# sovrasov/3d-object-detection.pytorch

Hardware: AMD Instinct MI355X
Metric: regression train crops/sec @224^2 bs256 MobileNetV2 (higher is better)
Workload: dtype bf16; 1 GPU; mobilenetv2 9-class Objectron keypoint regression, train step (fwd + l1/add/CE losses + bwd + AdamW), 224x224 crops, per-GPU batch 256; global_batch=256, parallelism=dp1, roofline_sampled_steps=0, rccl_ranks=0

## Files before the change

3d-object-detection.pytorch_amd/csrc/pwconv_wgrad_tr.hip:

```cpp
#include <cstdlib>
#include "pwconv_route.h"

namespace {

__device__ __forceinline__ f32x2 pk_fma_clamp01(f32x2 a, f32x2 b, f32x2 c) {
  f32x2 d;
  asm("v_pk_fma_f32 %0, %1, %2, %3 clamp" : "=v"(d) : "v"(a), "v"(b), "v"(c));
  return d;
}

typedef __attribute__((ext_vector_type(4))) short s16x4;

__device__ __forceinline__ void act_vec8(float* v, int act) {
  switch (act) {
    case T3D_ACT_RELU:
#pragma unroll
      for (int j = 0; j < 8; ++j) v[j] = fmaxf(v[j], 0.f);
      break;
    case T3D_ACT_RELU6:
#pragma unroll
      for (int j = 0; j < 8; ++j) v[j] = __builtin_amdgcn_fmed3f(v[j], 0.f, 6.f);
      break;
    case T3D_ACT_HSWISH:
#pragma unroll
// ... 9 lines not shown
  int per_sample;
  const float *scale, *shift, *se;
  int act, se_after;
  float* dw;
  int M, HW, K, N;
  int yfree, Nz;
  int swap;
  int ptiles, qtiles, rows_per_split, nsplit;
  float* ws;
  const T3dFold* fold;
  const bf16_t* wd;
  const bf16_t* wtr;
  const void *e_res, *e_y;
  void* dx;
  double* stats;
  int nrep;
  long long rstride;
  int unused_[10];
  int assign;
  int gs_ns;
  unsigned mulHW;
};

__device__ __forceinline__ bf16x8 tr_frag(const bf16_t* tile, int rs, int ch0, int lane) {
  const int g = lane >> 4, q = (lane & 15) >> 2, p = lane & 3;
  const bf16_t* a0 = tile + (8 * g + q) * rs + ch0 + 4 * p;
  const s16x4 lo = __builtin_amdgcn_ds_read_tr16_b64_v4i16((s16x4 __attribute__((address_space(3)))*)(a0));
  const s16x4 hi = __builtin_amdgcn_ds_read_tr16_b64_v4i16((s16x4 __attribute__((address_space(3)))*)(a0 + 4 * rs));
  typedef __attribute__((ext_vector_type(8))) short s16x8;
  const s16x8 v = {lo[0], lo[1], lo[2], lo[3], hi[0], hi[1], hi[2], hi[3]};
  return __builtin_bit_cast(bf16x8, v);
}

template <int NTPW, int NTQ, bool SWAP, int G, int D, int GEN, bool YF, int SK = 1, bool DGF = false>
__global__ __launch_bounds__(256 * G) void pw_wgrad_tr_kernel(const WgtArgs a) {
  static_assert(!DGF || (YF && !SWAP), "the fused data gradient exists for the y-free layout only");
  constexpr int PB = 64 * NTPW, QB = 16 * NTQ;
  constexpr int RSP = PB + 8, RSQ = QB + 8;
  constexpr int STEP = 32 * SK;
  extern __shared__ __attribute__((aligned(16))) unsigned char smem[];
  constexpr int BUFE = STEP * (RSP + RSQ);
  const int grp = threadIdx.x >> 8;
  bf16_t* const tiles = reinterpret_cast<bf16_t*>(smem) + grp * 2 * BUFE;
  float* coef = reinterpret_cast<float*>(reinterpret_cast<bf16_t*>(smem) + G * 2 * BUFE);
  constexpr int RSW = PB + 8;
  constexpr int NCOEF = 3 * (SWAP ? QB : PB) + 2 * (SWAP ? PB : QB);
  bf16_t* const wdl = reinterpret_cast<bf16_t*>(coef + ((NCOEF + 3) & ~3));
  double* const dstat = reinterpret_cast<double*>(wdl + (DGF ? QB * RSW : 0));

  const int tid = threadIdx.x & 255, lane = tid & 63, wave = tid >> 6;
  const int P = SWAP ? a.K : a.N, Q = SWAP ? a.N : a.K;
  const int ntiles = a.ptiles * a.qtiles, s8 = a.nsplit & ~7;
  int tile, split;
  {
    const int L = blockIdx.x;
    if (ntiles > 1 && L < ntiles * s8) {
      const int j = L >> 3;
      tile = j % ntiles;
      split = (j / ntiles) * 8 + (L & 7);
    } else {
      const int Lr = ntiles > 1 ? L - ntiles * s8 : L;
      tile = Lr % ntiles;
      split = (ntiles > 1 ? s8 : 0) + Lr / ntiles;
    }
  }
  const int pt = tile / a.qtiles, qt = tile % a.qtiles;
  const int p0 = pt * PB, q0 = qt * QB;
  const int mbeg = split * a.rows_per_split, mend = min(a.M, mbeg + a.rows_per_split);
  constexpr int dyB = SWAP ? QB : PB, aB = SWAP ? PB : QB;
// ... 94 lines not shown
#pragma unroll
            for (int r = 0; r < 4; ++r) {
              const int k = kt * 16 + 4 * lgq_ + r, k2 = qt2 * 16 + lcq_;
              if (k < K && k2 < K) wdl[k * RSW + Nz + k2] = (bf16_t)qa[r];
            }
          }
          __syncthreads();
        }
      if (grp == 0) {
        for (int kb = 0; kb < QB; kb += 16) {
          const int row = tid >> 4, sub = tid & 15, k = kb + row;
          float s2 = 0.f;
          if (k < K)
            for (int n = sub * 8; n < Nz; n += 128) {
              const bf16x8 v = *reinterpret_cast<const bf16x8*>(wtr + (size_t)k * Nz + n);
#pragma unroll
              for (int j = 0; j < 8; ++j) s2 = fmaf(gamma[n + j], (float)v[j], s2);
            }
          s2 = row16_sum(s2);
          if (sub == 0 && k < K) wdl[k * RSW + Nz + K] = (bf16_t)s2;
        }
      }
    }
    for (int i = threadIdx.x; i < 2 * QB; i += 256 * G) dstat[i] = 0.0;
  }
  const bf16_t* __restrict__ dz = reinterpret_cast<const bf16_t*>(a.dz);
  const bf16_t* __restrict__ yy = reinterpret_cast<const bf16_t*>(a.y);
  const bf16_t* __restrict__ xx = reinterpret_cast<const bf16_t*>(a.x);
  const bool plain_a = !a.scale && !a.se && a.act == T3D_ACT_NONE;

  constexpr int dyV = dyB / 8, aV = aB / 8;
  constexpr int ndv = STEP * dyV, nav = STEP * aV;
  constexpr int VDY = (ndv + 255) / 256, VA = (nav + 255) / 256;
  constexpr int NU = DGF ? (STEP / 16) * NTQ : 1, UPW = (NU + 3) / 4;
  struct Epi { bf16x4 res[UPW], xr[UPW]; };
  struct NoMask {};
  struct Regs { bf16x8 rz[VDY], ry[VDY], rx[VA]; Epi e; NoMask okm; };
  Regs rr[D];
  Epi ecur;
  const int lgq = lane >> 4, lcq = lane & 15;
  const bf16_t* __restrict__ eres = reinterpret_cast<const bf16_t*>(a.e_res);
  const bf16_t* __restrict__ eyr = reinterpret_cast<const bf16_t*>(a.e_y);

  auto gload = [&](Regs& R, int m0) {
#pragma unroll
    for (int i = 0; i < VDY; ++i) {
      const int v = min(tid + 256 * i, ndv - 1);
      const int row = v / dyV, m = min(m0 + row, a.M - 1);
      if constexpr (YF) {
        const int n = dy0 + (v % dyV) * 8;
        const bool fromz = n < a.Nz;
        const bf16_t* src = fromz ? dz + (size_t)m * a.Nz + n : xx + (size_t)m * a.K + min(max(n - a.Nz, 0), a.K - 8);
        R.rz[i] = *reinterpret_cast<const bf16x8*>(src);
      } else {
        const int n = min(dy0 + (v % dyV) * 8, a.N - 8);
        R.rz[i] = *reinterpret_cast<const bf16x8*>(dz + (size_t)m * a.N + n);
        R.ry[i] = *reinterpret_cast<const bf16x8*>(yy + (size_t)m * a.N + n);
      }
    }
#pragma unroll
    for (int i = 0; i < VA; ++i) {
      const int v = min(tid + 256 * i, nav - 1);
      const int row = v / aV, k = min(a0c + (v % aV) * 8, a.K - 8), m = min(m0 + row, a.M - 1);
      R.rx[i] = *reinterpret_cast<const bf16x8*>(xx + (size_t)m * a.K + k);
    }
    if constexpr (DGF) {
#pragma unroll
      for (int i = 0; i < UPW; ++i) {
        const int un = min(wave + 4 * i, NU - 1), pt = un / NTQ, kt = un % NTQ;
        const size_t o = (size_t)min(m0 + pt * 16 + lcq, a.M - 1) * a.K + min(kt * 16 + 4 * lgq, a.K - 4);
        if (eres) R.e.res[i] = *reinterpret_cast<const bf16x4*>(eres + o);
        if (eyr) R.e.xr[i] = *reinterpret_cast<const bf16x4*>(eyr + o);
      }
    }
  };
  auto ld8 = [](const float* p, float* o) {
    const float4 q0 = *reinterpret_cast<const float4*>(p), q1 = *reinterpret_cast<const float4*>(p + 4);
    o[0] = q0.x; o[1] = q0.y; o[2] = q0.z; o[3] = q0.w; o[4] = q1.x; o[5] = q1.y; o[6] = q1.z; o[7] = q1.w;
  };
  bf16x8 zero8;
#pragma unroll
  for (int j = 0; j < 8; ++j) zero8[j] = (bf16_t)0.f;
  auto lstore = [&](const Regs& R, int m0, int buf) {
    const auto& rz = R.rz; const auto& ry = R.ry; const auto& rx = R.rx;
    bf16_t* const pb_ = tiles + buf * BUFE;
    bf16_t* const qb_ = pb_ + STEP * RSP;
    bf16_t* dyt = SWAP ? qb_ : pb_;
    bf16_t* at = SWAP ? pb_ : qb_;
    constexpr int rsd = SWAP ? RSQ : RSP, rsa = SWAP ? RSP : RSQ;
#pragma unroll
    for (int i = 0; i < VDY; ++i) {
      const int v = tid + 256 * i;
      if (v < ndv) {
        const int row = v / dyV, cl = (v % dyV) * 8, m = m0 + row;
        const bool ok = m < mend && dy0 + cl < a.N;
        bf16x8 o;
        if constexpr (YF) {
          const int n = dy0 + cl;
          o = rz[i];
          if (n >= a.Nz + a.K) {
            o = zero8;
            if (n == a.Nz + a.K) o[0] = (bf16_t)1.f;
          }
          *reinterpret_cast<bf16x8*>(dyt + row * rsd + cl) = ok ? o : zero8;
          continue;
        }
        float al[8], be[8], ga[8];
        ld8(cdy + dyB + cl, be);
        if constexpr (GEN == 1) {
          if (a.per_sample) {
            const size_t pb = (size_t)(min(m, a.M - 1) / a.HW) * a.N + min(dy0 + cl, a.N - 8);
#pragma unroll
            for (int j = 0; j < 8; ++j) { al[j] = a.alpha[pb + j]; ga[j] = a.gamma[pb + j]; }
          } else {
            ld8(cdy + cl, al);
            ld8(cdy + 2 * dyB + cl, ga);
          }
        } else {
          ld8(cdy + cl, al);
          ld8(cdy + 2 * dyB + cl, ga);
        }
#pragma unroll
        for (int j = 0; j < 8; ++j) o[j] = (bf16_t)fmaf(al[j], (float)rz[i][j], fmaf(be[j], (float)ry[i][j], ga[j]));
        *reinterpret_cast<bf16x8*>(dyt + row * rsd + cl) = ok ? o : zero8;
// ... 30 lines not shown
          }
          if constexpr (GEN == 1) {
            if (a.se) {
              float svv[8];
              {
                const float* se = a.se + (size_t)(min(m, a.M - 1) / a.HW) * a.K + min(a0c + cl, a.K - 8);
#pragma unroll
                for (int j = 0; j < 8; ++j) svv[j] = se[j];
              }
#pragma unroll
              for (int j = 0; j < 8; ++j) {
                float t = fmaf(u[j], sc[j], sh[j]);
                const float sv = svv[j];
                if (!a.se_after) t *= sv;
                t = act_apply(t, a.act);
                if (a.se_after) t *= sv;
                u[j] = t;
              }
              done = true;
            }
          }
          if (c6) {
#pragma unroll
            for (int j = 0; j < 8; j += 2) {
              const f32x2 t = pk_fma_clamp01(f32x2{u[j], u[j + 1]}, f32x2{sc[j], sc[j + 1]}, f32x2{sh[j], sh[j + 1]});
              u[j] = t[0];
              u[j + 1] = t[1];
            }
          } else if (!done) act_affine_vec<8>(u, sc, sh, a.act);
#pragma unroll
          for (int j = 0; j < 8; ++j) o[j] = (bf16_t)u[j];
        }
        *reinterpret_cast<bf16x8*>(at + row * rsa + cl) = ok ? o : zero8;
      }
    }
  };

  f32x4 acc[NTPW][NTQ];
#pragma unroll
  for (int i = 0; i < NTPW; ++i)
#pragma unroll
    for (int j = 0; j < NTQ; ++j) acc[i][j] = f32x4{0.f, 0.f, 0.f, 0.f};
  float st1[UPW][4], st2[UPW][4];
#pragma unroll
  for (int i = 0; i < UPW; ++i)
#pragma unroll
    for (int r = 0; r < 4; ++r) st1[i][r] = st2[i][r] = 0.f;
  auto dgrad_step = [&](const bf16_t* pcur, int m0) {
    bf16_t* __restrict__ dxo = reinterpret_cast<bf16_t*>(a.dx);
#pragma unroll
    for (int i = 0; i < UPW; ++i) {
      const int un = wave + 4 * i;
      if (un < NU) {
        const int pt = un / NTQ, kt = un % NTQ;
        f32x4 d = {0.f, 0.f, 0.f, 0.f};
#pragma unroll
        for (int js = 0; js < PB / 32; ++js) {
          const bf16x8 af = *reinterpret_cast<const bf16x8*>(wdl + (kt * 16 + lcq) * RSW + js * 32 + 8 * lgq);
          const bf16x8 bfr = *reinterpret_cast<const bf16x8*>(pcur + (pt * 16 + lcq) * RSP + js * 32 + 8 * lgq);
          d = __builtin_amdgcn_mfma_f32_16x16x32_bf16(af, bfr, d, 0, 0, 0);
        }
        const int m = m0 + pt * 16 + lcq, k = kt * 16 + 4 * lgq;
        const bool ok = m < mend && k < a.K;
        float v[4] = {d[0], d[1], d[2], d[3]}, yv[4] = {0.f, 0.f, 0.f, 0.f};
        if (eres) {
#pragma unroll
          for (int r = 0; r < 4; ++r) v[r] += (float)ecur.res[i][r];
        }
        bf16x4 o;
#pragma unroll
        for (int r = 0; r < 4; ++r) {
          o[r] = (bf16_t)v[r];
          v[r] = ok ? (float)o[r] : 0.f;
        }
        if (ok) *reinterpret_cast<bf16x4*>(dxo + (size_t)m * a.K + k) = o;
        if (a.stats) {
#pragma unroll
          for (int r = 0; r < 4; ++r) {
            if (eyr) yv[r] = (float)ecur.xr[i][r];
            st1[i][r] += v[r];
            st2[i][r] = fmaf(v[r], eyr ? yv[r] : v[r], st2[i][r]);
          }
        }
      }
    }
  };

  __syncthreads();
  const int nsteps = (mend - mbeg + STEP - 1) / STEP;
  const int niter = (nsteps + G - 1) / G;
  auto step_m = [&](int it) { return mbeg + (it * G + grp) * STEP; };
#pragma unroll
  for (int u = 0; u < D; ++u) gload(rr[u], step_m(u));
  lstore(rr[0], step_m(0), 0);
  if constexpr (DGF) ecur = rr[0].e;
  __syncthreads();
  int buf = 0;
  for (int it0 = 0; it0 < niter; it0 += D) {
#pragma unroll
    for (int u = 0; u < D; ++u) {
      const int it = it0 + u;
      if (it < niter) {
        gload(rr[u], step_m(it + D));
        const bf16_t* pcur = tiles + buf * BUFE;
        const bf16_t* qcur = pcur + STEP * RSP;
#pragma unroll
        for (int kk = 0; kk < SK; ++kk) {
          bf16x8 qf[NTQ];
#pragma unroll
          for (int j = 0; j < NTQ; ++j) qf[j] = tr_frag(qcur + kk * 32 * RSQ, RSQ, j * 16, lane);
#pragma unroll
          for (int i = 0; i < NTPW; ++i) {
            const bf16x8 pf = tr_frag(pcur + kk * 32 * RSP, RSP, (wave + 4 * i) * 16, lane);
#pragma unroll
            for (int j = 0; j < NTQ; ++j) acc[i][j] = __builtin_amdgcn_mfma_f32_16x16x32_bf16(pf, qf[j], acc[i][j], 0, 0, 0);
          }
        }
        if constexpr (DGF) {
          dgrad_step(pcur, step_m(it));
          ecur = rr[(u + 1) % D].e;
// ... 104 lines not shown
  if (sp == 0 && live) dw[(size_t)p * K + q] = assign ? s : dw[(size_t)p * K + q] + s;
}

template <int SG>
__global__ __launch_bounds__(256) void wgrad_reduce_tr_kernel(const float* __restrict__ ws, float* __restrict__ dw, int N, int K,
                                                               int PB, int QB, int qtiles, int tiles, int S, int assign) {
  constexpr int PT = 8 / SG;
  __shared__ float part[8][33];
  const int Qpad = qtiles * QB, nq = (Qpad + 31) / 32;
  const int p0 = (blockIdx.x / nq) * PT, q0 = (blockIdx.x % nq) * 32;
  const int tx = threadIdx.x & 31, rest = threadIdx.x >> 5, sg = rest / PT, pl = rest % PT;
  const size_t stride = (size_t)tiles * PB * QB;
  const int q = q0 + tx, p = p0 + pl;
  float s = 0.f;
  if (p < K && q < N) {
    const float* src = ws + (size_t)((p / PB) * qtiles + q / QB) * (PB * QB) + (size_t)(p % PB) * QB + q % QB;
#pragma unroll 8
    for (int i = sg; i < S; i += SG) s += src[(size_t)i * stride];
  }
  part[rest][tx] = s;
  __syncthreads();
  if (threadIdx.x < 32 * PT) {
    const int pl2 = threadIdx.x % PT, ql = threadIdx.x / PT;
    const int k = p0 + pl2, n = q0 + ql;
    if (k < K && n < N) {
      float t = part[pl2][ql];
#pragma unroll
      for (int g = 1; g < SG; ++g) t += part[g * PT + pl2][ql];
      dw[(size_t)n * K + k] = assign ? t : dw[(size_t)n * K + k] + t;
    }
  }
}

template <int NTPW, int NTQ, bool SWAP, int D, int GEN, bool YF = false, int SK = 1>
int launch_d(WgtArgs& a, hipStream_t st) {
  constexpr int G = 2;
  constexpr int STEP = 32 * SK;
  constexpr int PB = 64 * NTPW, QB = 16 * NTQ;
  const int P = a.swap ? a.K : a.N, Q = a.swap ? a.N : a.K;
  a.ptiles = cdiv(P, PB);
  a.qtiles = cdiv(Q, QB);
  const int tiles = a.ptiles * a.qtiles;
  const int dyB = a.swap ? QB : PB, aB = a.swap ? PB : QB;
  size_t lds = (size_t)G * 2 * STEP * ((PB + 8) + (QB + 8)) * 2 + (size_t)(3 * dyB + 2 * aB) * 4;
  const int tgt_blocks = 256;
  const long long cap_mb = 8;
  int S = (tgt_blocks + tiles - 1) / tiles;
  const long long tile_bytes = (long long)tiles * PB * QB * 4;
  const bool use_ws = g_t3d_ws.ptr && g_t3d_ws.bytes >= tile_bytes;
  if (use_ws) {
    const long long fit = g_t3d_ws.bytes / tile_bytes;
    if (S > fit) S = (int)fit;
  } else {
    const long long flush_cap = (cap_mb << 20) / ((long long)a.N * a.K * 4 + 1);
    if (S > flush_cap) S = (int)(flush_cap < 1 ? 1 : flush_cap);
  }
  const int maxs = cdiv(a.M, STEP * 4 * G);
  if (S > maxs) S = maxs;
  if (S < 1) S = 1;
  a.rows_per_split = cdiv(cdiv(a.M, S), STEP) * STEP;
  S = cdiv(a.M, a.rows_per_split);
  a.gs_ns = 0;
  if constexpr (GEN == 2) {
    const long long ns = a.rows_per_split / a.HW + 2, span = (long long)a.rows_per_split + a.HW;
    if (!a.se || a.per_sample || a.HW < 2 || ns * aB * 4 > 32 * 1024 || span * a.HW >= (1ll << 32)) return launch_d<NTPW, NTQ, SWAP, 1, 1>(a, st);
    a.gs_ns = (int)ns;
    a.mulHW = (unsigned)(((1ull << 32) + a.HW - 1) / a.HW);
    lds = ((lds + 15) & ~(size_t)15) + (size_t)ns * aB * 4;
  }
  a.ws = use_ws ? reinterpret_cast<float*>(g_t3d_ws.ptr) : nullptr;
  if (a.assign && !use_ws && hipMemsetAsync(a.dw, 0, (size_t)a.N * a.K * sizeof(float), st) != hipSuccess) return T3D_ERR_LAUNCH;
  if (lds > 64 * 1024)
    (void)t3d_max_lds((const void*)pw_wgrad_tr_kernel<NTPW, NTQ, SWAP, G, D, GEN, YF, SK, false>, (int)lds);
  a.nsplit = S;
  T3D_LAUNCH_TIMED((pw_wgrad_tr_kernel<NTPW, NTQ, SWAP, G, D, GEN, YF, SK, false>), dim3(tiles * S), dim3(256 * G), lds, st, a);
  if (use_ws) {
#define T3D_WGR(SPV)                                                                                                              \
  do {                                                                                                                            \
    if (SWAP)                                                                                                                     \
      T3D_LAUNCH(wgrad_reduce_tr_kernel<(SPV == 16 ? 8 : SPV)>, dim3(cdiv(a.K, 8 / (SPV == 16 ? 8 : SPV)) * cdiv(a.qtiles * QB, 32)), dim3(256), 0, st, \
                         a.ws, a.dw, a.N, a.K, PB, QB, a.qtiles, tiles, S, a.assign);                                             \
    else                                                                                                                          \
      T3D_LAUNCH(wgrad_reduce_kernel<SPV>, dim3(cdiv(a.N * a.qtiles * QB, 256 / SPV)), dim3(256), 0, st, a.ws, a.dw, a.N, \
                         a.K, PB, QB, a.qtiles, tiles, S, a.assign);                                                              \
  } while (0)
    if (S >= 64) T3D_WGR(16);
    else if (S >= 8) T3D_WGR(4);
    else T3D_WGR(1);
#undef T3D_WGR
  }
  T3D_CHECK_LAUNCH();
  return T3D_OK;
}

template <int NTPW, int NTQ, bool SWAP>
int launch_sw(WgtArgs& a, hipStream_t st) {
  constexpr bool narrow = 64 * NTPW + 16 * NTQ <= 288;
  const bool sk2 = narrow && a.M >= (1 << 20);
  if (a.yfree) {
    if constexpr (SWAP) return T3D_ERR_ARG;
    else {
      if constexpr (narrow)
        if (sk2) return launch_d<NTPW, NTQ, false, 2, false, true, 2>(a, st);
      return launch_d<NTPW, NTQ, false, 2, false, true>(a, st);
    }
  }
  if (a.per_sample) return launch_d<NTPW, NTQ, SWAP, 1, 1>(a, st);
  if (a.se) return launch_d<NTPW, NTQ, SWAP, 2, 2>(a, st);
  if constexpr (narrow)
    if (sk2) return launch_d<NTPW, NTQ, SWAP, 2, false, false, 2>(a, st);
  return launch_d<NTPW, NTQ, SWAP, 2, false>(a, st);
}

template <int NTPW, int NTQ>
int launch_cfg(WgtArgs& a, hipStream_t st) {
  return a.swap ? launch_sw<NTPW, NTQ, true>(a, st) : launch_sw<NTPW, NTQ, false>(a, st);
}

static int choose_and_launch(WgtArgs& a, hipStream_t st) {
  const int M = a.M, K = a.K, N = a.N;
  a.swap = K > N;
  const int P = a.swap ? K : N, Q = a.swap ? N : K;
  const int min_steps = 12;
  auto steps_with = [&](int ntpw, int qb) {
    const int tiles = cdiv(P, 64 * ntpw) * cdiv(Q, qb);
    int S = cdiv(256, tiles);
    if (S < 1) S = 1;
    return M / (S * 2 * 32);
  };
  if (Q <= 16) return (P <= 64 || steps_with(2, 16) < min_steps) ? launch_cfg<1, 1>(a, st) : launch_cfg<2, 1>(a, st);
  if (Q <= 32) {
    if (P <= 64 || steps_with(3, 32) < min_steps) return launch_cfg<1, 2>(a, st);
    return P <= 128 ? launch_cfg<2, 2>(a, st) : launch_cfg<3, 2>(a, st);
  }
// ... 130 lines not shown
```

3d-object-detection.pytorch_amd/torchdet3d/models/engine.py:

```python
import contextlib
import math
import os

import torch

from .. import _native as N
from .arch import Arch

BN_EPS, BN_MOM = 1e-5, 0.1
NREP = 16
FUSED_EVAL_MIN_B = int(os.environ.get('T3D_FUSED_EVAL_MIN_B', '96'))
DW_SLOTS = 512
WORKSPACE_BYTES = 64 << 20
MAIN_WORKSPACE_BYTES = 16 << 20
YFREE_MIN_ELEMS = int(os.environ.get('T3D_YFREE_MIN', 8 << 20))
YFREE_MAX_K = 112
HOOK_MIN = 1 << 20
SE_AFTER_FUSED = None


def _se_after_fused_by_shape(dt, B, HW, C, R):
    if B < 8:
        return False
    if C * R <= 4096:
        return True
    return B >= 16 and B * HW >= 1024


class _BN:
    __slots__ = ('name', 'C', 'gamma', 'beta', 'dgamma', 'dbeta', 'rm', 'rv', 'nbt', 'stats', 'bstats', 'scale',
                 'shift', 'mean', 'invstd', 'alpha', 'bbeta', 'gammac', 'count', 'pro_cache', 'pend', 'desc', 'nrep')


def _nrep_for(C):
    return 16 if C <= 160 else (8 if C <= 640 else 4)


def _concurrent_stream(device, tries=8):
    main = torch.cuda.current_stream(device)
    cands = []
    with torch.cuda.device(device):
        probe = torch.zeros(1, device=device)
        for _ in range(tries):
            st = torch.cuda.Stream(device=device, priority=0)
            cands.append(st)
            e0, e_side, e_main = (torch.cuda.Event(enable_timing=True) for _ in range(3))
            torch.cuda.synchronize(device)
            e0.record(main)
            torch.cuda._sleep(4_000_000)
# ... 32 lines not shown
        self.feat_gain = 1.0
        if self.arch.head == 'conv_bias':
            self.pool = N.POOL['avg']
            self.feat_gain = 2.0 if pooling_mode == 'avg+max' else 1.0
        self.device = torch.device(device)
        assert dtype in (torch.float32, torch.bfloat16, torch.float16)
        self.dtype = dtype
        self.dt = {torch.float32: N.F32, torch.bfloat16: N.BF16, torch.float16: N.F16}[dtype]
        self.esz = 4 if dtype == torch.float32 else 2
        self._share = share
        self._layout()
        self._bufs = {}
        self._packed_dirty = True
        self._packed_version = -1
        self._pack_desc = self._se_pack_desc = None
        self._evdesc = None
        self._dwarena = self._zero_rows = None
        self._zgroups = {'fwd': {}, 'bwd': {}}
        self._zcovered = {'fwd': frozenset(), 'bwd': frozenset()}
        self._zgdesc, self._zdescs = {}, {}
        self._want_taps = None
        self._stop_after = None
        self._tap_res = {}
        self._dropout_calls = 0
        self.seed_rank = 0
        self.saved = None
        self.generation = 0
        self.grad_hook = None
        self._cur_pool_exact = False
        self._side = None
        if self.device.type == 'cuda' and not os.environ.get('T3D_NO_SIDE_STREAM'):
            self._side = _concurrent_stream(self.device)
        self._side_busy = False
        self.persistent_outputs = False
        self.set_input_normalization([0.5931, 0.4690, 0.4229], [0.2471, 0.2214, 0.2157])
        self._fused_eval = True

    def set_input_normalization(self, mean, std):
        self.in_mean = torch.tensor(mean, dtype=torch.float32, device=self.device)
        self.in_istd = 1.0 / torch.tensor(std, dtype=torch.float32, device=self.device)

    def _layout(self):
        a = self.arch
        shapes = a.param_shapes(self.num_classes)
        self.shapes = shapes
        order = [k for k, (s, kind) in shapes.items() if kind == 'param' and not k.startswith('regressors.')]
        off, self.offsets = 0, {}
        for k in order:
            n = int(math.prod(shapes[k][0]))
            self.offsets[k] = (off, n)
            off += (n + 3) // 4 * 4
        F = a.feat_c
        self.offsets['__wreg'] = (off, 9 * 18 * F)
        off += 9 * 18 * F
        self.offsets['__breg'] = (off, 9 * 18 + 2)
        off += 164
        for k in range(9):
            self.offsets[f'regressors.{k}.0.weight'] = (self.offsets['__wreg'][0] + k * 18 * F, 18 * F)
            self.offsets[f'regressors.{k}.0.bias'] = (self.offsets['__breg'][0] + k * 18, 18)
        self.nparams = off
        dev = self.device
        sh = self._share
        assert sh is None or (sh.nparams == off and sh.name == self.name and sh.device == dev)
        self.flat = sh.flat if sh is not None else torch.zeros(off, device=dev)
        self.gflat = sh.gflat if sh is not None else torch.zeros(off, device=dev)
        self.p, self.g = {}, {}
# ... 331 lines not shown
            N.call('t3d_set_main_workspace', N.ptr(ws), MAIN_WORKSPACE_BYTES)
        else:
            N.call('t3d_set_main_workspace', None, 0)

    @contextlib.contextmanager
    def _pass(self, main_scratch=False, workspace=False):
        self._cur_nrep = None
        self._replicas(NREP)
        if workspace:
            N.call('t3d_set_workspace', N.ptr(self._buf('workspace', (WORKSPACE_BYTES,), torch.uint8)), WORKSPACE_BYTES)
        if main_scratch:
            self._main_scratch(True)
        try:
            yield
        finally:
            N.call('t3d_set_reduction_replicas', 1, 0)
            if workspace:
                N.call('t3d_set_dw_slots', 0, None)
            self._pool_exact(False)
            self._cur_nrep = None
            if workspace:
                N.call('t3d_set_workspace', None, 0)
            if main_scratch:
                self._main_scratch(False)

    def forward(self, imgs, cats, train=False, dropout_mask=None, all_heads=False):
        with self._pass(main_scratch=True):
            return self._forward(imgs, cats, train, dropout_mask, all_heads)

    def _forward(self, imgs, cats, train=False, dropout_mask=None, all_heads=False):
        a, st = self.arch, N.stream()
        if train and self.dt == N.F16:
            raise RuntimeError('fp16 storage is an inference-only mode (build the model with storage_dtype bf16 or f32 to train)')
        sv = self._features(imgs, train)
        B = sv['B']
        pooled, cur, yl, prol = sv['pooled'], sv['last_in'], sv['yl'], sv['prol']
        if not all_heads:
            cats = cats.to(self.device, torch.int64).contiguous()
        sv['cats'] = cats
        amax = None
        if self.pool != N.POOL['avg']:
            amax = self._buf('pool_argmax', (B, a.last_c), torch.int32)
        self._c('t3d_pool_fwd', self.dt, N.ptr(yl), prol, self.pool, N.ptr(pooled), N.ptr(amax), B, cur.H * cur.W,
                a.last_c, st, fwd=sv['bnl'])
        sv['pool_argmax'] = amax

        f, fpro = pooled, None
        if a.head == 'linear_bn':
            bnc = self.bns[a.keys.head_bn]
            yc = self._buf('y:cls', (B, a.classifier), torch.float32)
            N.call('t3d_pwconv_fwd', N.F32, N.ptr(pooled), None, N.ptr(self.p[a.keys.head_w]),
                   N.ptr(self.p[a.keys.head_b]), N.ptr(yc), self._st(bnc), B, 1, a.last_c, a.classifier, st)
            fpro = self._bn_fwd(bnc, B, 'hswish')
            self._settle_f(bnc)
            f = yc
        elif a.head == 'conv_bias':
            Fc = a.classifier
            yc = self._buf('y:cls', (B, Fc), torch.float32)
            N.call('t3d_pwconv_fwd', N.F32, N.ptr(pooled), None, N.ptr(self.p[a.keys.head_w]),
                   N.ptr(self.p[a.keys.head_b]), N.ptr(yc), None, B, 1, a.last_c, Fc, st)
            f, fpro = yc, N.prologue(self._const(Fc, 1.0), self._const(Fc, 0.0), None, 'hswish', False)
            sv['head_u'], sv['head_pro'] = yc, fpro
            if self.feat_gain != 1.0:
                f = self._buf('f:gain', (B, Fc), torch.float32)
                N.call('t3d_bn_apply', N.F32, N.ptr(yc), fpro, None, N.ptr(f), B, Fc, st)
                N.call('t3d_bn_apply', N.F32, N.ptr(f), None, N.ptr(f), N.ptr(f), B, Fc, st)
                fpro = None
        ncls = self.num_classes
        keep = self.persistent_outputs
        logits = (self._buf('out:logits', (B, ncls), torch.float32) if keep else torch.empty(B, ncls, device=self.device)) if ncls > 1 else None
        if all_heads:
            kp = self._buf('out:kp_all', (9, B, 18), torch.float32) if keep else torch.empty(9, B, 18, device=self.device)
            N.call('t3d_head_fwd_all', N.ptr(f), fpro, N.ptr(self.wreg), N.ptr(self.breg),
                   N.ptr(self.p['cls_fc.1.weight']) if ncls > 1 else None,
                   N.ptr(self.p['cls_fc.1.bias']) if ncls > 1 else None, N.ptr(kp), N.ptr(logits), B, a.feat_c, ncls, st)
            self.saved = None
            return kp.view(9, B, 9, 2), logits
        mask = None
        if train and ncls > 1:
            mask = dropout_mask
            if mask is None:
                mask = self._buf('dropout', (B, a.feat_c), torch.float32)
                self._dropout_calls += 1
                seed = (torch.initial_seed() + 0x9E3779B97F4A7C15 * self.seed_rank) & ((1 << 64) - 1)
                N.call('t3d_dropout_mask', N.ptr(mask), B * a.feat_c, seed, self._dropout_calls, 0.5, st, slots={3: N.SLOT_DROPOUT})
            else:
                mask = mask.to(self.device, torch.float32).contiguous()
        kp = self._buf('out:kp', (B, 18), torch.float32) if keep else torch.empty(B, 18, device=self.device)
        N.call('t3d_head_fwd', N.ptr(f), fpro, N.ptr(cats), N.ptr(self.wreg), N.ptr(self.breg),
               N.ptr(self.p['cls_fc.1.weight']), N.ptr(self.p['cls_fc.1.bias']), N.ptr(mask), N.ptr(kp),
               N.ptr(logits), B, a.feat_c, ncls, st)
        sv.update(f=f, fpro=fpro, mask=mask, kp=kp)
        assert not any(b.pend[0] for b in self.bns.values()), 'a BatchNorm finalize was never run'
        if train:
            self.generation += 1
            sv['generation'] = self.generation
        self.saved = sv if train else None
        return kp.view(B, 9, 2), logits

    def forward_taps(self, imgs, tap_blocks):
        self._want_taps = set(tap_blocks)
        try:
            with self._pass():
                sv = self._features(imgs, False)
        finally:
            self._want_taps = None
        return {k: (s.t, s.B, s.H, s.W, s.C) for k, s in sv['taps'].items()}

    def _check_train_taps(self, taps):
        a = self.arch
        if a.kind != 'mobilenet' or not taps or min(taps) < 1 or max(taps) > len(a.blocks):
            raise NotImplementedError(f'tapped training pass: taps {sorted(taps)} of {self.name}')
        for k in sorted(taps)[:-1]:
            blk = a.blocks[k]
            if blk.res or not blk.expand:
                why = 'has a skip connection' if blk.res else 'has no expansion'
                raise NotImplementedError(f'tapped training pass: the tap at features.{k} feeds features.{k + 1}, which {why}')

    def forward_taps_train(self, imgs, tap_blocks):
        taps = set(int(k) for k in tap_blocks)
        self._check_train_taps(taps)
# ... 34 lines not shown
        s = sv['taps'][deep]
        M = s.B * s.H * s.W
        dz = self._buf('dz:tap', (M, s.C))
        N.call('t3d_bn_act_bwd', self.dt, N.ptr(dtaps[deep]), N.ptr(s.raw), None, N.ptr(dz), self._bst(s.bn), M, s.C, st)
        self._tap_res = {k: dtaps[k] for k in order[:-1]}
        try:
            for rec in reversed(sv['blocks']):
                dz = self._block_bwd(rec, dz)
                self._maybe_hook(self.offsets[a.keys.blocks[rec['idx']].first][0])
        finally:
            self._tap_res = {}
        self._stem_wgrad(sv, dz, dw32)
        self._flush_dw()
        self._join_side()
        self._maybe_hook(0, force=True)
        assert not any(b.pend[1] for b in self.bns.values()), 'a BatchNorm backward finalize was never run'
        self.saved = None

    def extract_features(self, imgs):
        with self._pass():
            sv = self._features(imgs, False)
        cur, a = sv['last_in'], self.arch
        M = sv['B'] * cur.H * cur.W
        z = torch.empty(M, a.last_c, device=self.device, dtype=self.dtype)
        N.call('t3d_bn_apply', self.dt, N.ptr(sv['yl']), sv['prol'], None, N.ptr(z), M, a.last_c, N.stream())
        return z.float().view(sv['B'], cur.H, cur.W, a.last_c).permute(0, 3, 1, 2).contiguous()

    def _features(self, imgs, train):
        a, st, dt = self.arch, N.stream(), self.dt
        u8 = imgs.dtype == torch.uint8
        assert imgs.is_cuda and imgs.dim() == 4 and ((u8 and imgs.shape[3] == 3) or (imgs.dtype == torch.float32 and imgs.shape[1] == 3))
        imgs = imgs.contiguous()
        self.training = bool(train)
        self._pack()
        if u8:
            B, H, W, _ = imgs.shape
        else:
            B, _, H, W = imgs.shape
        if train:
            self._zero_group('fwd', [[self._statbuf.data_ptr(), self._statbuf.numel() * self._statbuf.element_size()]])
        else:
            self._zero_group('fwd')
            self._eval_affines()
        sv = dict(B=B, imgs=imgs, blocks=[])
        self.saved_blocks = sv['blocks']

        Ho, Wo = (H + 2 - 3) // 2 + 1, (W + 2 - 3) // 2 + 1
        M = B * Ho * Wo
        bn0 = self.bns[a.keys.stem_bn]
        y0 = self._buf('y:stem', (M, a.stem_c))
        col = self._buf('col', (M, 32))
        if u8:
            N.call('t3d_stem_im2col_u8', dt, N.ptr(imgs), N.ptr(self.in_mean), N.ptr(self.in_istd), N.ptr(col), B, H, W, st)
        else:
            N.call('t3d_stem_im2col', dt, N.ptr(imgs), N.ptr(col), B, H, W, st)
        N.call('t3d_pwconv_fwd', dt, N.ptr(col), None, N.ptr(self.w['stem']), None, N.ptr(y0), self._st(bn0),
               M, Ho * Wo, 32, a.stem_c, st, nbytes=M * (32 + a.stem_c) * self.esz)
        pro0 = self._bn_fwd(bn0, M, a.stem_act)
        cur = _Src(y0, pro0, B, Ho, Wo, a.stem_c, raw=y0, bn=bn0, gpro=pro0)
        sv['col'], sv['stem'] = col, cur

        taps = self._want_taps
        for i, blk in enumerate(a.blocks):
            cur = self._block_fwd(i, blk, cur, sv)
            if taps and (i + 1) in taps:
                sv.setdefault('taps', {})[i + 1] = self._resolve(cur)
            if self._stop_after == i + 1:
                return sv

        bnl = self.bns[a.keys.last_bn]
        M = cur.B * cur.H * cur.W
        yl = self._buf('y:last', (M, a.last_c))
        self._pw_from(cur, self.w[a.keys.last_w], yl, bnl, M, cur.H * cur.W, cur.C, a.last_c)
        prol = self._bn_fwd(bnl, M, a.last_act)
        pooled = self._buf('pooled', (B, a.last_c), torch.float32)
        sv.update(last_in=cur, yl=yl, prol=prol, pooled=pooled, HWl=cur.H * cur.W, bnl=bnl)
        return sv

    def _wsel(self, w, plain=True):
        f = self._frag.get(w.data_ptr()) if (plain and self.dt in (N.BF16, N.F16)) else None
        return (self.dt | N.W_FRAG, N.ptr(f)) if f is not None else (self.dt, N.ptr(w))

    def _resolve(self, src):
        if src.zbuf is not None:
            M = src.B * src.H * src.W
            self._c('t3d_bn_apply', self.dt, N.ptr(src.t), src.pro, N.ptr(src.zres), N.ptr(src.zbuf), M, src.C, N.stream(),
                    fwd=src.bn)
            src.t, src.pro, src.zres, src.zbuf = src.zbuf, None, None, None
# ... 147 lines not shown
        if ro is not None and ro.pend[1] and not req:
            self._settle_b(ro)
        if req:
            N.call('t3d_fold_request', N.ptr(self._fold_desc(ro, 1, ro.count)), N.ptr(ro.alpha))
        try:
            self._wgrad_issue(entry, args, kw)
        finally:
            if req and N.lib().t3d_fold_pending():
                raise RuntimeError(f'{entry} left a BatchNorm finalize request unserved (engine / library mismatch)')

    def _wgrad_issue(self, entry, args, kw):
        if self._side is None:
            N.call(entry, *args, N.stream(), **kw)
            return
        self._fork_side()
        if N.timer is None:
            N.call(entry, *args, self._side.cuda_stream, **kw)
        else:
            with torch.cuda.stream(self._side):
                N.call(entry, *args, N.stream(), **kw)
        self._side_busy = True

    def _se_wgrad(self, se, sen, dq, dp, B, C, R):
        self._wgrad(N.ptr(se['m']), N.ptr(se['h']), N.ptr(dq), N.ptr(dp), N.ptr(self.g[sen.se_w1]),
                    N.ptr(self.g[sen.se_b1]), N.ptr(self.g[sen.se_w2]), N.ptr(self.g[sen.se_b2]),
                    B, C, R, entry='t3d_se_bwd_weights')

    def _fork_side(self):
        main = torch.cuda.current_stream()
        self._side.wait_stream(main)
        if N.recorder is not None:
            N.recorder.add_fork(main.cuda_stream, self._side.cuda_stream)

    def _join_side(self):
        if self._side is not None and self._side_busy:
            main = torch.cuda.current_stream()
            main.wait_stream(self._side)
            if N.recorder is not None:
                N.recorder.add_fork(self._side.cuda_stream, main.cuda_stream)
            self._side_busy = False

    def backward(self, dkp, dlogits=None):
        with self._pass(main_scratch=True, workspace=True):
            return self._backward(dkp, dlogits)

    def _clear_backward(self):
        if self._dwarena is None:
            self._dw_arena_init()
        dw32 = self._buf('dstem32', (self.arch.stem_c, 32), torch.float32)
        if self._zero_rows is None:
            rows = [[t.data_ptr(), t.numel() * t.element_size()] for t in (self.gflat, dw32) if t.numel()]
            rows += [[v.data_ptr(), NREP * self.p[k].numel() * 4] for k, v in self._dwviews.items()]
            assert all(r[1] % 16 == 0 for r in rows)
            self._zero_rows = rows
        self._zero_group('bwd', self._zero_rows)
        return dw32

    def _backward(self, dkp, dlogits=None):
        sv = self.saved
        assert sv is not None and 'tap_order' not in sv, 'backward() needs a preceding forward(train=True)'
        a, st, dt, B = self.arch, N.stream(), self.dt, sv['B']
        dw32 = self._clear_backward()
        self._dwpending, self._dwflushed, self._hook_hi = 0, 0, self.gflat.numel()
        dkp = dkp.reshape(B, 18).to(torch.float32).contiguous()
        ncls = self.num_classes
        if ncls > 1:
            assert dlogits is not None
            dlogits = dlogits.to(torch.float32).contiguous()
        else:
            dlogits = None
        F = a.feat_c
        dpre = self._buf('dpre', (B, 18), torch.float32)
        df = self._buf('df', (B, F), torch.float32)
        bnc = self.bns[a.keys.head_bn] if a.head == 'linear_bn' else None
        hstat = None
        if a.head == 'conv_bias':
            hstat = self._buf('head_stats', (2 * F,), torch.float64, zgroup='bwd')
            self._replicas(1)
        N.call('t3d_head_bwd', N.ptr(sv['f']), sv['fpro'], N.ptr(sv['cats']), N.ptr(self.wreg),
               N.ptr(self.p['cls_fc.1.weight']), N.ptr(sv['mask']), N.ptr(sv['kp']), N.ptr(dkp), N.ptr(dlogits),
               N.ptr(dpre), N.ptr(df), self._bst(bnc) if bnc else (N.ptr(hstat) if sv['fpro'] is not None else None),
               None, None, None, None, B, F, ncls, st)
        self._wgrad(N.ptr(sv['f']), sv['fpro'], N.ptr(sv['cats']), N.ptr(sv['mask']), N.ptr(dpre), N.ptr(dlogits),
                    N.ptr(self.dwreg), N.ptr(self.dbreg), N.ptr(self.g['cls_fc.1.weight']), N.ptr(self.g['cls_fc.1.bias']),
                    B, F, ncls, entry='t3d_head_bwd_weights')
        dpooled = df
        if a.head == 'conv_bias':
            yc, pooled, Fc = sv['head_u'], sv['pooled'], a.classifier
            if sv['fpro'] is None:
                du = self._buf('dhead_u', (B, Fc), torch.float32)
                N.call('t3d_bn_act_bwd', N.F32, N.ptr(df), N.ptr(yc), sv['head_pro'], N.ptr(du), N.ptr(hstat), B, Fc, st)
                df = du
            gain, zeros = self._const(Fc, self.feat_gain), self._const(Fc, 0.0)
            bb = N.bnbwd(gain, zeros, zeros, False)
            self._wgrad(N.F32, N.ptr(df), N.ptr(yc), bb, N.ptr(pooled), None, N.ptr(self.g[a.keys.head_w]), B, 1, a.last_c, Fc)
# ... 21 lines not shown
        self.saved = None

    def _backward_backbone(self, sv, dpooled, dw32):
        a, st, dt, B = self.arch, N.stream(), self.dt, sv['B']
        lw = a.keys.last_w
        bnl = self.bns[a.keys.last_bn]
        x = sv['last_in']
        M, HW = B * sv['HWl'], sv['HWl']
        dzl = self._buf('dz:last', (M, a.last_c))
        N.call('t3d_pool_bwd', dt, N.ptr(dpooled), N.ptr(sv['yl']), sv['prol'], self.pool, N.ptr(sv['pool_argmax']),
               N.ptr(dzl), self._bst(bnl), B, HW, a.last_c, st)
        bb = self._bn_bwd(bnl)
        def last_wgrad():
            self._wgrad(dt, N.ptr(dzl), N.ptr(sv['yl']), bb, N.ptr(x.t), x.pro,
                        N.ptr(self.g[lw]), M, HW, x.C, a.last_c, nbytes=M * (x.C + a.last_c) * self.esz,
                        ro=bnl)
        last_wgrad()
        dz = self._pw_dgrad(dzl, sv['yl'], bb, self.wt[lw], x, None, M, HW, x.C, a.last_c, 'dz:lastin', bnl)

        self._maybe_hook(self.offsets[lw][0])
        for rec in reversed(sv['blocks']):
            dz = self._block_bwd(rec, dz)
            self._maybe_hook(self.offsets[a.keys.blocks[rec['idx']].first][0])

        self._stem_wgrad(sv, dz, dw32)

    def _stem_wgrad(self, sv, dz, dw32):
        a, st, dt = self.arch, N.stream(), self.dt
        s0 = sv['stem']
        bn0 = s0.bn
        bb = self._bn_bwd(bn0)
        self._settle_b(bn0)
        M = s0.B * s0.H * s0.W
        self._wgrad(dt, N.ptr(dz), N.ptr(s0.raw), bb, N.ptr(sv['col']), None, N.ptr(dw32),
                    M, s0.H * s0.W, 32, a.stem_c, nbytes=M * (32 + a.stem_c) * self.esz)
        self._flush_dw()
        self._join_side()
        N.call('t3d_copy_cols', N.ptr(dw32), N.ptr(self.g[a.keys.stem_w]), a.stem_c, 32, 27, st)

    def _pw_dgrad(self, dz, y, bb, wt, x, residual, M, HW, K, Nn, tag, bn=None):
        dx = self._buf(tag, (M, K))
        with_stats = x.bn is not None and not x.finished_act
        wd, wp = self._wsel(wt, not bb.per_sample and not (with_stats and x.gpro is not None and x.gpro.se))
        self._c('t3d_pwconv_dgrad', wd, N.ptr(dz), N.ptr(y), bb, wp,
                N.ptr(x.raw) if with_stats else None, x.gpro if with_stats else None,
                N.ptr(residual) if residual is not None else None, N.ptr(dx),
                self._bst(x.bn) if with_stats else None, None, M, HW, K, Nn, N.stream(),
                nbytes=M * (K + Nn) * self.esz, bwd=bn)
        if x.finished_act:
            dx = self._act_bwd(dx, x, tag + ':a')
        return dx

    def _dw_arena_init(self):
        names = [k for k, (sh, kind) in self.shapes.items() if kind == 'param' and len(sh) == 4 and sh[1] == 1 and sh[2] > 1]
        tot = sum(DW_SLOTS * self.p[k].numel() for k in names)
        self._dwarena = torch.zeros(tot, device=self.device, dtype=torch.float32)
        self._dwused = torch.zeros(max(len(names), 1), device=self.device, dtype=torch.int32)
        self._dwviews, self._dwidx, off = {}, {}, 0
        for k in names:
            n = self.p[k].numel()
            self._dwviews[k] = self._dwarena[off:off + DW_SLOTS * n]
            off += DW_SLOTS * n
        self._dworder = list(reversed(names))
        rows = []
        for i, k in enumerate(self._dworder):
            self._dwidx[k] = i
            rows.append([self._dwviews[k].data_ptr(), self.g[k].data_ptr(), self.p[k].numel(), self._dwused[i:i + 1].data_ptr()])
        self._dwdesc = torch.tensor(rows, dtype=torch.int64, device=self.device) if rows else None
# ... 198 lines not shown
```

3d-object-detection.pytorch_amd/torchdet3d/trainer/step_plan.py:

```python
import ctypes
import os

import torch

from .. import _native as N

WARM_STEPS = 2
REPLAY = os.environ.get('T3D_STEP_PLAN', '1') != '0'


class StepPlan:
    def __init__(self, model, loss_manager, optimizer):
        self.model, self.lm, self.opt = model, loss_manager, optimizer
        self.rec = None
        self.key = None
        self.warm = 0
        self.slots = (ctypes.c_ulonglong * N.NSLOTS)()
        self.replays = 0

    @staticmethod
    def usable(model, lm, opt):
        from ..builders.model_builder import ModelWrapper
        from ..builders.optim_builder import FusedOptimizer
        if not isinstance(model, ModelWrapper) or model.export_mode or model.net.device.type != 'cuda':
            return False
        if lm is None or not getattr(lm, '_fused', False) or lm.use_alwa:
            return False
        if not isinstance(opt, FusedOptimizer) or len(opt.param_groups) != 1:
            return False
        ps = opt.param_groups[0]['params']
        return len(ps) == 1 and ps[0] is model.flat

    def accepts(self, imgs, gt_kp, cats):
        m = self.model
        if not (m.training and torch.is_grad_enabled() and N.timer is None):
            return False
        B = imgs.shape[0]
        return (imgs.is_cuda and imgs.is_contiguous() and imgs.dtype in (torch.float32, torch.uint8) and imgs.dim() == 4
                and gt_kp.is_cuda and gt_kp.dtype == torch.float32 and gt_kp.is_contiguous() and gt_kp.numel() == B * 18
                and cats.is_cuda and cats.dtype == torch.int64 and cats.is_contiguous() and cats.numel() == B
                and imgs.device == m.net.device)

    def _key(self, imgs):
        net = self.model.net
        return (id(net), tuple(imgs.shape), imgs.dtype, N.stream(), id(net._side), bytes(self.lm.loss_cfg()),
                self.opt.plan_key(self.model.flat, self.opt.param_groups[0]), torch.initial_seed(),
                id(net.grad_hook), net.num_classes)

    def run(self, imgs, gt_kp, cats, slot):
        key = self._key(imgs)
        if key != self.key:
            self._drop()
            self.key, self.warm = key, 0
        if self.rec is not None and REPLAY:
            return self._replay(imgs, gt_kp, cats, slot), True
        record = REPLAY and self.warm >= WARM_STEPS
        out = self._direct(imgs, gt_kp, cats, record)
        self.warm += 1
        return out, False

    def _drop(self):
        if self.rec is not None:
            self.rec.close()
            self.rec = None

    def __del__(self):
        try:
            self._drop()
        except Exception:
            pass

    def _bufs(self, B):
        net = self.model.net
        ncls = net.num_classes
        out = net._buf('loss:out', (16,), torch.float32)
        dkp = net._buf('loss:dkp', (B, 18), torch.float32)
        dlg = net._buf('loss:dlg', (B, ncls), torch.float32, zero=('loss:dlg', (B, ncls), torch.float32) not in net._bufs) if ncls > 1 else None
        return out, dkp, dlg

    def _direct(self, imgs, gt_kp, cats, record):
# ... 246 lines not shown
```

Baseline: 38790 crops/s.

## Overlap stem im2col, dropout mask and grad clear on side stream; y-free stem wgrad

The stem im2col gather, the dropout mask generation and the backward gradient-arena clear now run on the side stream during forward, so they overlap with weight packing and BN stat zeroing. The stem weight gradient uses the y-free wgrad path with a new compact-staging kernel variant (ZV) for Nz=K=32, which loads dz directly and reuses the loaded activation as the x part. This removes the recompute of y and its extra reads. In exchange it adds stream fork/join points, a new template instantiation and extra LDS zero-fill, and it changes the step-plan key.

```diff
diff --git a/3d-object-detection.pytorch_amd/csrc/pwconv_wgrad_tr.hip b/3d-object-detection.pytorch_amd/csrc/pwconv_wgrad_tr.hip
--- a/3d-object-detection.pytorch_amd/csrc/pwconv_wgrad_tr.hip
+++ b/3d-object-detection.pytorch_amd/csrc/pwconv_wgrad_tr.hip
@@ -65,9 +65,10 @@
   return __builtin_bit_cast(bf16x8, v);
 }
 
-template <int NTPW, int NTQ, bool SWAP, int G, int D, int GEN, bool YF, int SK = 1, bool DGF = false>
+template <int NTPW, int NTQ, bool SWAP, int G, int D, int GEN, bool YF, int SK = 1, bool DGF = false, int ZV = 0>
 __global__ __launch_bounds__(256 * G) void pw_wgrad_tr_kernel(const WgtArgs a) {
   static_assert(!DGF || (YF && !SWAP), "the fused data gradient exists for the y-free layout only");
+  static_assert(ZV == 0 || (YF && !SWAP && !DGF && !GEN && 8 * ZV < 64 * NTPW), "compact staging: the plain y-free products only");
   constexpr int PB = 64 * NTPW, QB = 16 * NTQ;
   constexpr int RSP = PB + 8, RSQ = QB + 8;
   constexpr int STEP = 32 * SK;
@@ -228,6 +229,8 @@
   constexpr int dyV = dyB / 8, aV = aB / 8;
   constexpr int ndv = STEP * dyV, nav = STEP * aV;
   constexpr int VDY = (ndv + 255) / 256, VA = (nav + 255) / 256;
+  constexpr int nzv = STEP * ZV, VZ = (nzv + 255) / 256;
+  static_assert(VZ <= VDY, "");
   constexpr int NU = DGF ? (STEP / 16) * NTQ : 1, UPW = (NU + 3) / 4;
   struct Epi { bf16x4 res[UPW], xr[UPW]; };
   struct NoMask {};
@@ -239,8 +242,16 @@
   const bf16_t* __restrict__ eyr = reinterpret_cast<const bf16_t*>(a.e_y);
 
   auto gload = [&](Regs& R, int m0) {
-#pragma unroll
-    for (int i = 0; i < VDY; ++i) {
+    if constexpr (ZV > 0) {
+#pragma unroll
+      for (int i = 0; i < VZ; ++i) {
+        const int v = min(tid + 256 * i, nzv - 1);
+        const int m = min(m0 + v / ZV, a.M - 1);
+        R.rz[i] = *reinterpret_cast<const bf16x8*>(dz + (size_t)m * a.Nz + (v % ZV) * 8);
+      }
+    }
+#pragma unroll
+    for (int i = 0; i < (ZV > 0 ? 0 : VDY); ++i) {
       const int v = min(tid + 256 * i, ndv - 1);
       const int row = v / dyV, m = min(m0 + row, a.M - 1);
       if constexpr (YF) {
@@ -284,8 +295,23 @@
     bf16_t* dyt = SWAP ? qb_ : pb_;
     bf16_t* at = SWAP ? pb_ : qb_;
     constexpr int rsd = SWAP ? RSQ : RSP, rsa = SWAP ? RSP : RSQ;
-#pragma unroll
-    for (int i = 0; i < VDY; ++i) {
+    if constexpr (ZV > 0) {
+#pragma unroll
+      for (int i = 0; i < VZ; ++i) {
+        const int v = tid + 256 * i;
+        if (v < nzv) {
+          const int row = v / ZV;
+          *reinterpret_cast<bf16x8*>(dyt + row * rsd + (v % ZV) * 8) = m0 + row < mend ? rz[i] : zero8;
+        }
+      }
+      if (tid < STEP) {
+        bf16x8 o = zero8;
+        if (m0 + tid < mend) o[0] = (bf16_t)1.f;
+        *reinterpret_cast<bf16x8*>(dyt + tid * rsd + a.Nz + a.K) = o;
+      }
+    }
+#pragma unroll
+    for (int i = 0; i < (ZV > 0 ? 0 : VDY); ++i) {
       const int v = tid + 256 * i;
       if (v < ndv) {
         const int row = v / dyV, cl = (v % dyV) * 8, m = m0 + row;
@@ -382,6 +408,9 @@
           for (int j = 0; j < 8; ++j) o[j] = (bf16_t)u[j];
         }
         *reinterpret_cast<bf16x8*>(at + row * rsa + cl) = ok ? o : zero8;
+        if constexpr (ZV > 0) {
+          if (cl < a.K) *reinterpret_cast<bf16x8*>(dyt + row * rsd + a.Nz + cl) = ok ? rx[i] : zero8;
+        }
       }
     }
   };
@@ -436,6 +465,13 @@
     }
   };
 
+  if constexpr (ZV > 0) {
+    const int c0 = a.Nz + a.K + 8, nz8 = (PB - c0) / 8;
+    for (int i = tid; i < 2 * STEP * nz8; i += 256) {
+      const int r = i / nz8;
+      *reinterpret_cast<bf16x8*>(tiles + (r / STEP) * BUFE + (r % STEP) * RSP + c0 + (i % nz8) * 8) = zero8;
+    }
+  }
   __syncthreads();
   const int nsteps = (mend - mbeg + STEP - 1) / STEP;
   const int niter = (nsteps + G - 1) / G;
@@ -606,7 +642,7 @@
   }
 }
 
-template <int NTPW, int NTQ, bool SWAP, int D, int GEN, bool YF = false, int SK = 1>
+template <int NTPW, int NTQ, bool SWAP, int D, int GEN, bool YF = false, int SK = 1, int ZV = 0>
 int launch_d(WgtArgs& a, hipStream_t st) {
   constexpr int G = 2;
   constexpr int STEP = 32 * SK;
@@ -645,9 +681,9 @@
   a.ws = use_ws ? reinterpret_cast<float*>(g_t3d_ws.ptr) : nullptr;
   if (a.assign && !use_ws && hipMemsetAsync(a.dw, 0, (size_t)a.N * a.K * sizeof(float), st) != hipSuccess) return T3D_ERR_LAUNCH;
   if (lds > 64 * 1024)
-    (void)t3d_max_lds((const void*)pw_wgrad_tr_kernel<NTPW, NTQ, SWAP, G, D, GEN, YF, SK, false>, (int)lds);
+    (void)t3d_max_lds((const void*)pw_wgrad_tr_kernel<NTPW, NTQ, SWAP, G, D, GEN, YF, SK, false, ZV>, (int)lds);
   a.nsplit = S;
-  T3D_LAUNCH_TIMED((pw_wgrad_tr_kernel<NTPW, NTQ, SWAP, G, D, GEN, YF, SK, false>), dim3(tiles * S), dim3(256 * G), lds, st, a);
+  T3D_LAUNCH_TIMED((pw_wgrad_tr_kernel<NTPW, NTQ, SWAP, G, D, GEN, YF, SK, false, ZV>), dim3(tiles * S), dim3(256 * G), lds, st, a);
   if (use_ws) {
 #define T3D_WGR(SPV)                                                                                                              \
   do {                                                                                                                            \
@@ -674,6 +710,8 @@
   if (a.yfree) {
     if constexpr (SWAP) return T3D_ERR_ARG;
     else {
+      if constexpr (NTPW == 2 && NTQ == 2)
+        if (sk2 && a.Nz == 32 && a.K == 32) return launch_d<2, 2, false, 2, false, true, 2, 4>(a, st);
       if constexpr (narrow)
         if (sk2) return launch_d<NTPW, NTQ, false, 2, false, true, 2>(a, st);
       return launch_d<NTPW, NTQ, false, 2, false, true>(a, st);
diff --git a/3d-object-detection.pytorch_amd/torchdet3d/models/engine.py b/3d-object-detection.pytorch_amd/torchdet3d/models/engine.py
--- a/3d-object-detection.pytorch_amd/torchdet3d/models/engine.py
+++ b/3d-object-detection.pytorch_amd/torchdet3d/models/engine.py
@@ -15,6 +15,7 @@
 MAIN_WORKSPACE_BYTES = 16 << 20
 YFREE_MIN_ELEMS = int(os.environ.get('T3D_YFREE_MIN', 8 << 20))
 YFREE_MAX_K = 112
+STEM_YFREE = True
 HOOK_MIN = 1 << 20
 SE_AFTER_FUSED = None
 
@@ -113,6 +114,8 @@
         if self.device.type == 'cuda' and not os.environ.get('T3D_NO_SIDE_STREAM'):
             self._side = _concurrent_stream(self.device)
         self._side_busy = False
+        self._side_fwd = None
+        self.side_input = True
         self.persistent_outputs = False
         self.set_input_normalization([0.5931, 0.4690, 0.4229], [0.2471, 0.2214, 0.2157])
         self._fused_eval = True
@@ -510,7 +513,12 @@
         a, st = self.arch, N.stream()
         if train and self.dt == N.F16:
             raise RuntimeError('fp16 storage is an inference-only mode (build the model with storage_dtype bf16 or f32 to train)')
-        sv = self._features(imgs, train)
+        if train and not all_heads and self.side_input and self._side is not None and self.grad_hook is None:
+            self._side_fwd = dict(mask=self.num_classes > 1 and dropout_mask is None)
+        try:
+            sv = self._features(imgs, train)
+        finally:
+            self._side_fwd = None
         B = sv['B']
         pooled, cur, yl, prol = sv['pooled'], sv['last_in'], sv['yl'], sv['prol']
         if not all_heads:
@@ -555,7 +563,9 @@
             self.saved = None
             return kp.view(9, B, 9, 2), logits
         mask = None
-        if train and ncls > 1:
+        if 'mask' in sv:
+            mask = sv['mask']
+        elif train and ncls > 1:
             mask = dropout_mask
             if mask is None:
                 mask = self._buf('dropout', (B, a.feat_c), torch.float32)
@@ -565,6 +575,7 @@
             else:
                 mask = mask.to(self.device, torch.float32).contiguous()
         kp = self._buf('out:kp', (B, 18), torch.float32) if keep else torch.empty(B, 18, device=self.device)
+        self._join_side()
         N.call('t3d_head_fwd', N.ptr(f), fpro, N.ptr(cats), N.ptr(self.wreg), N.ptr(self.breg),
                N.ptr(self.p['cls_fc.1.weight']), N.ptr(self.p['cls_fc.1.bias']), N.ptr(mask), N.ptr(kp),
                N.ptr(logits), B, a.feat_c, ncls, st)
@@ -665,11 +676,26 @@
         assert imgs.is_cuda and imgs.dim() == 4 and ((u8 and imgs.shape[3] == 3) or (imgs.dtype == torch.float32 and imgs.shape[1] == 3))
         imgs = imgs.contiguous()
         self.training = bool(train)
-        self._pack()
         if u8:
             B, H, W, _ = imgs.shape
         else:
             B, _, H, W = imgs.shape
+        Ho, Wo = (H + 2 - 3) // 2 + 1, (W + 2 - 3) // 2 + 1
+        M = B * Ho * Wo
+        col = self._buf('col', (M, 32))
+
+        def gather():
+            if u8:
+                N.call('t3d_stem_im2col_u8', dt, N.ptr(imgs), N.ptr(self.in_mean), N.ptr(self.in_istd), N.ptr(col), B, H, W, N.stream())
+            else:
+                N.call('t3d_stem_im2col', dt, N.ptr(imgs), N.ptr(col), B, H, W, N.stream())
+        side = self._side_fwd
+        if side is not None:
+            self._fork_side()
+            with torch.cuda.stream(self._side):
+                gather()
+            self._side_busy = True
+        self._pack()
         if train:
             self._zero_group('fwd', [[self._statbuf.data_ptr(), self._statbuf.numel() * self._statbuf.element_size()]])
         else:
@@ -678,15 +704,13 @@
         sv = dict(B=B, imgs=imgs, blocks=[])
         self.saved_blocks = sv['blocks']
 
-        Ho, Wo = (H + 2 - 3) // 2 + 1, (W + 2 - 3) // 2 + 1
-        M = B * Ho * Wo
         bn0 = self.bns[a.keys.stem_bn]
         y0 = self._buf('y:stem', (M, a.stem_c))
-        col = self._buf('col', (M, 32))
-        if u8:
-            N.call('t3d_stem_im2col_u8', dt, N.ptr(imgs), N.ptr(self.in_mean), N.ptr(self.in_istd), N.ptr(col), B, H, W, st)
+        if side is None:
+            gather()
         else:
-            N.call('t3d_stem_im2col', dt, N.ptr(imgs), N.ptr(col), B, H, W, st)
+            self._join_side()
+            self._side_early(sv, side)
         N.call('t3d_pwconv_fwd', dt, N.ptr(col), None, N.ptr(self.w['stem']), None, N.ptr(y0), self._st(bn0),
                M, Ho * Wo, 32, a.stem_c, st, nbytes=M * (32 + a.stem_c) * self.esz)
         pro0 = self._bn_fwd(bn0, M, a.stem_act)
@@ -900,6 +924,24 @@
         if N.recorder is not None:
             N.recorder.add_fork(main.cuda_stream, self._side.cuda_stream)
 
+    def _side_early(self, sv, what):
+        a, B = self.arch, sv['B']
+        mask = self._buf('dropout', (B, a.feat_c), torch.float32) if what['mask'] else None
+        clear = torch.is_grad_enabled()
+        if clear and self._dwarena is None:
+            self._dw_arena_init()
+        with torch.cuda.stream(self._side):
+            if mask is not None:
+                self._dropout_calls += 1
+                seed = (torch.initial_seed() + 0x9E3779B97F4A7C15 * self.seed_rank) & ((1 << 64) - 1)
+                N.call('t3d_dropout_mask', N.ptr(mask), B * a.feat_c, seed, self._dropout_calls, 0.5, N.stream(),
+                       slots={3: N.SLOT_DROPOUT})
+            if clear:
+                sv['dw32'] = self._clear_backward()
+        if what['mask']:
+            sv['mask'] = mask
+        self._side_busy = True
+
     def _join_side(self):
         if self._side is not None and self._side_busy:
             main = torch.cuda.current_stream()
@@ -928,7 +970,9 @@
         sv = self.saved
         assert sv is not None and 'tap_order' not in sv, 'backward() needs a preceding forward(train=True)'
         a, st, dt, B = self.arch, N.stream(), self.dt, sv['B']
-        dw32 = self._clear_backward()
+        dw32 = sv.pop('dw32', None)
+        if dw32 is None:
+            dw32 = self._clear_backward()
         self._dwpending, self._dwflushed, self._hook_hi = 0, 0, self.gflat.numel()
         dkp = dkp.reshape(B, 18).to(torch.float32).contiguous()
         ncls = self.num_classes
@@ -1016,8 +1060,12 @@
         bb = self._bn_bwd(bn0)
         self._settle_b(bn0)
         M = s0.B * s0.H * s0.W
-        self._wgrad(dt, N.ptr(dz), N.ptr(s0.raw), bb, N.ptr(sv['col']), None, N.ptr(dw32),
-                    M, s0.H * s0.W, 32, a.stem_c, nbytes=M * (32 + a.stem_c) * self.esz)
+        if dt == N.BF16 and STEM_YFREE and 0 < YFREE_MIN_ELEMS <= M * a.stem_c:
+            self._wgrad(N.ptr(dz), N.ptr(sv['col']), bb, N.ptr(self.w['stem']), N.ptr(dw32), M, s0.H * s0.W, 32, a.stem_c,
+                        entry='t3d_pwconv_wgrad_yfree', nbytes=M * (32 + a.stem_c) * self.esz)
+        else:
+            self._wgrad(dt, N.ptr(dz), N.ptr(s0.raw), bb, N.ptr(sv['col']), None, N.ptr(dw32),
+                        M, s0.H * s0.W, 32, a.stem_c, nbytes=M * (32 + a.stem_c) * self.esz)
         self._flush_dw()
         self._join_side()
         N.call('t3d_copy_cols', N.ptr(dw32), N.ptr(self.g[a.keys.stem_w]), a.stem_c, 32, 27, st)
diff --git a/3d-object-detection.pytorch_amd/torchdet3d/trainer/step_plan.py b/3d-object-detection.pytorch_amd/torchdet3d/trainer/step_plan.py
--- a/3d-object-detection.pytorch_amd/torchdet3d/trainer/step_plan.py
+++ b/3d-object-detection.pytorch_amd/torchdet3d/trainer/step_plan.py
@@ -45,7 +45,7 @@
         net = self.model.net
         return (id(net), tuple(imgs.shape), imgs.dtype, N.stream(), id(net._side), bytes(self.lm.loss_cfg()),
                 self.opt.plan_key(self.model.flat, self.opt.param_groups[0]), torch.initial_seed(),
-                id(net.grad_hook), net.num_classes)
+                id(net.grad_hook), net.num_classes, net.side_input)
 
     def run(self, imgs, gt_kp, cats, slot):
         key = self._key(imgs)
```

After: 38770 crops/s (median of 2 runs). About the same (-0.0%).
